# shgaurav1/DVG

Measured on AMD Instinct MI355X. Metric: predicted frames/sec at 64x64, batch 64, 10-in/10-out, higher is better.
Workload: dtype f32; 1 GPU; Moving-MNIST 64x64 rollout (generate_frames.py make_gifs sample loop), vgg_64 + lstm + GP trigger sample at i%15==0, batch 64 per GPU, 10-in/10-out; model_family=vgg, batch_per_gpu=64, n_past=10, n_future=10, parallelism=replicas x1 (no data-path collective), launch=hipGraph replay, rollouts_in_flight=3, tile_policy=energy, loop_invariant_skip_halves=hoisted, upsample_conv3x3=as transposed 4x4/s2 conv, conv3x3_deep_layers=Winograd F(4x4,3x3) / F(2x2,3x3)

## Files before the change

### dvg_amd/csrc/conv_igemm2.hip

```cpp
#include <cstdlib>
#include <type_traits>

#include "dvg_common.h"

namespace dvg {

constexpr int DVG_GEMM_WGS_PER_CU = DVG_BF16X3 ? 3 : 4;
constexpr int DVG_GEMM128_WGS = DVG_BF16X3 ? 3 : 2;
constexpr int DVG_GEMM128_GT = DVG_BF16X3 ? 2 : 4;
constexpr int DVG_GEMM_GT = 4;
constexpr int DVG_GEMM128_MIN_WGS = 4 * 768;
[[maybe_unused]] constexpr int DVG_GEMM_NT2 = 256;
constexpr int DVG_TILE16_MIN_WGS = 256;

enum { M2_CONV3 = 0, M2_CONV4S2 = 1, M2_CONVT4S2 = 2, M2_GEMM = 3 };

struct Igemm2Params {
    const float* x = nullptr;
    const float* skip = nullptr;
    const float* w = nullptr;
    const float* scale = nullptr;
    const float* shift = nullptr;
    float* y = nullptr;
    float* y_pool = nullptr;
    float* stats = nullptr;
    int N = 0, H = 0, W = 0, C1 = 0, C2 = 0, Cout = 0, upsample = 0, act = 0;
    float slope = 0.f;
    int tiles_y = 0, tiles_x = 0, tiles_n = 0, nblk_n = 0;
    int splitk = 1;
    int cps = 0;
    float* ws = nullptr;
    const float* addend = nullptr;
    unsigned long long* clk = nullptr;
    unsigned clk_cap = 0;
    int nb_group = 0;
    int stage_prio = 0;
    long w_image_stride = 0;
    int gemm_ni = 0;
    const int* add_map = nullptr;
    int add_B = 0;
    const float* first_frame = nullptr;
    const float* first_w = nullptr;
    const float* first_scale = nullptr;
    const float* first_shift = nullptr;
    float first_slope = 0.f;
    int y_from = 0;
    const float* proj_w = nullptr;
    float* proj_out = nullptr;
    int proj_T = 0;
};

__device__ __forceinline__ int addend_image(const int* __restrict__ add_map, int add_B, int n) {
    return add_map ? add_map[n / add_B] * add_B + n % add_B : n;
}

static unsigned long long* g_clk = nullptr;
static unsigned g_clk_cap = 0;

__device__ __attribute__((aligned(16))) float dvg_zero_slot[4] = {0.f, 0.f, 0.f, 0.f};

template <int MODE, int TI, int TH, int TW, int NT_ = 1, bool FIRST_ = false, bool PROJ_ = false>
struct Cfg2 {
    static constexpr int NT = NT_;
    static constexpr bool FIRST = FIRST_;
    static constexpr bool PROJ = PROJ_;
    static constexpr bool GEMM = MODE == M2_GEMM;
    static constexpr int S = (MODE == M2_CONV4S2) ? 2 : 1;
    static constexpr bool PAR4 = MODE == M2_CONV4S2;
    static constexpr int SPAN = GEMM ? 1 : (PAR4 ? 2 : 3);
    static constexpr int HH = (TH - 1) + SPAN, HW = (TW - 1) + SPAN;
    static constexpr bool LAYOUT = !GEMM;
    static constexpr int HWP = !LAYOUT ? HW : (TW == 16 ? HW : (TW == 8 ? 12 : 6));
    static constexpr int IMG = (LAYOUT && TI == 4) ? (PAR4 ? 30 : 40) : HH * HWP;
    static_assert(IMG >= HH * HWP && HWP >= HW, "halo layout");
    static constexpr int HP = TI * IMG;
    static constexpr unsigned P0PACK = !LAYOUT ? 0x6420u
        : (PAR4 ? (TW == 16 ? 0x3650u : (TI == 4 ? 0x7430u : 0x6530u))
                : (TW == 16 ? 0x2640u : (TI == 4 ? 0x6530u : 0x4620u)));
    static constexpr int PK = !LAYOUT ? 1 : (PAR4 ? (TW == 16 ? 4 : 1) : (TW == 16 ? 5 : (TI == 4 ? 1 : 3)));
    static constexpr bool STORE_PERM = LAYOUT && DVG_BF16X3 != 0;
    static constexpr int hp_of(int slot) {
        return STORE_PERM ? ((slot & ~7) | (((slot & 3) << 1) | ((slot >> 2) & 1))) : slot;
    }
    static constexpr int row_c(int reg) { return 4 * (int)((P0PACK >> (4 * (reg >> 2))) & 15u) + (reg & 3); }
    static constexpr int BM = TI * TH * TW, MT = BM / 64, BN = 64 * NT;
    static constexpr int NTAPS = GEMM ? 1 : ((MODE == M2_CONV3) ? 9 : 16);
    static constexpr int GT = (MODE == M2_CONV3) ? 9 : (MODE == M2_CONV4S2 ? 4 : (GEMM ? (NT == 2 ? 2 : (BM == 128 ? DVG_GEMM128_GT : DVG_GEMM_GT)) : 4));
    static constexpr int NG = (MODE == M2_CONV4S2) ? 16 / GT : 1;
    static constexpr int CHUNKS_PER_STAGE = GEMM ? GT : 1;
    static constexpr bool X3 = DVG_BF16X3 != 0;
    static constexpr int KC = 16, LD = X3 ? (GEMM ? 24 : 28) : 20, LDB = X3 ? 24 : 20, WROW = DVG_WROW;
    static constexpr int NP = X3 ? 3 : 2, PSTEP = X3 ? 8 : 4;
    static constexpr int BLK4 = GT * 64 * WROW / 4;
    static constexpr int B_TILE4 = NT * BLK4;
    static constexpr int NLB = (B_TILE4 + 255) / 256;
    static_assert(NT == 1 || (DVG_BF16X3 != 0 && MODE == M2_GEMM && BLK4 % 256 == 0), "NT = 2: bf16-triple GEMM mode only");
    static constexpr int NLA1 = (HP * 4 + 255) / 256;
    static constexpr int NLA = NLA1 * (GEMM ? GT : 1);
    static constexpr int SLAB = NLA1 * 64 * LD;
    static constexpr int A_FLOATS = NLA * 64 * LD, B_FLOATS = GT * BN * LDB;
    static constexpr int FP_W = HW + 2, FP_FLOATS = (HH + 2) * FP_W, FIRST_FLOATS = FIRST ? FP_FLOATS : 0;
    static_assert(!FIRST || (MODE == M2_CONV3 && TI == 1 && NT == 1), "FIRST: 3x3 mode, one image per tile");
    static constexpr int LDS_BYTES = (A_FLOATS + B_FLOATS + FIRST_FLOATS) * 4;
    static constexpr bool CAN_SPLIT = !FIRST && !GEMM && TW != 16 && !PROJ;
    static_assert(BM == 64 || BM == 128 || BM == 256, "BM");
    static_assert(!PROJ || (MODE == M2_CONVT4S2 && TI == 1 && NT == 1 && !FIRST && BM * 64 <= A_FLOATS + B_FLOATS),
                  "PROJ: transposed-conv mode, one image per tile, the staged tile fits the stage buffers");
};

template <int MODE, int TI, int TH, int TW, int NT = 1, bool FIRST = false, bool PROJ = false>
__global__ __launch_bounds__(256, (MODE == M2_GEMM && TW == 8) ? DVG_GEMM_WGS_PER_CU : ((MODE == M2_GEMM && NT == 1) ? DVG_GEMM128_WGS : 2)) void conv_igemm2_kernel(const Igemm2Params p) {
    using C = Cfg2<MODE, TI, TH, TW, NT, FIRST, PROJ>;
    constexpr int S = C::S, HH = C::HH, HW = C::HW, HP = C::HP, LD = C::LD, MT = C::MT, GT = C::GT, NG = C::NG,
                  BN = C::BN, NLA = C::NLA, NLA1 = C::NLA1, LDB = C::LDB, NP = C::NP, PSTEP = C::PSTEP, NLB = C::NLB;
    constexpr bool GEMM = C::GEMM, X3 = C::X3;
    extern __shared__ __attribute__((aligned(16))) float smem[];
    float* As = smem;
    float* Bs = smem + C::A_FLOATS;

    const int tid = threadIdx.x, lane = tid & 63, wave = tid >> 6;
    const int wm = wave >> 1, wn = wave & 1, l31 = lane & 31, hh = lane >> 5;

    unsigned lid = xcd_remap(blockIdx.x, gridDim.x);
    int par = 0;
    if (MODE == M2_CONVT4S2) { par = lid & 3; lid >>= 2; }
    const int split = lid % p.splitk;
    lid /= p.splitk;
    const int tiles_total = p.tiles_x * p.tiles_y * p.tiles_n;
    const unsigned lr = lid / p.nb_group;
    const int nb = (int)(lr / tiles_total) * p.nb_group + (int)(lid % p.nb_group);
    const unsigned tile_id = lr % tiles_total;
    unsigned t = tile_id;
    const int tx_i = t % p.tiles_x; t /= p.tiles_x;
    const int ty_i = t % p.tiles_y; t /= p.tiles_y;
    const int n0 = (int)t * (MODE == M2_GEMM ? p.gemm_ni : TI), y0 = ty_i * TH, x0 = tx_i * TW;
    const int yin0 = y0 * S - (GEMM ? 0 : 1), xin0 = x0 * S - (GEMM ? 0 : 1), nb0 = nb * BN;
    const float* const wbase = p.w + (GEMM ? (size_t)n0 * p.w_image_stride : 0);
    const int py = par >> 1, px = par & 1;
    const int Cin = p.C1 + p.C2;

    int a_base[MT];
#pragma unroll
    for (int mt = 0; mt < MT; ++mt) {
        const int lp = 4 * ((int)((C::P0PACK >> (4 * (l31 >> 3))) & 15u) ^ (((l31 >> 2) & 1) * C::PK)) + (l31 & 3);
        const int m = wm * (C::BM / 2) + mt * 32 + lp;
        const int ti = m / (TH * TW), r = m % (TH * TW);
        const int pos = ti * C::IMG + (r / TW) * C::HWP + r % TW;
        a_base[mt] = pos * LD + (X3 ? (hh ^ (GEMM ? (pos >> 3) & 1 : 0)) * 4 : hh * 8);
    }
    int b_base[NT];
#pragma unroll
    for (int nt = 0; nt < NT; ++nt) {
        const int col = (wn * NT + nt) * 32 + l31;
        b_base[nt] = ((col >> 6) * GT * 64 + (col & 63)) * LDB + (X3 ? (hh ^ ((l31 >> 3) & 1)) * 4 : hh * 8);
    }

    f32x16 acc[MT * NT];
#pragma unroll
    for (int mt = 0; mt < MT * NT; ++mt)
#pragma unroll
        for (int i = 0; i < 16; ++i) acc[mt][i] = 0.f;

    constexpr int NOFF = GEMM ? NLA1 : NLA;
    using aoff_t = typename std::conditional<GEMM || C::PAR4, int, long>::type;
    auto opaque = [](unsigned v) { asm("" : "+v"(v)); return v; };
    aoff_t offx[NOFF], offs[GEMM ? 1 : NLA];
    unsigned okmask = 0;
    static_assert(!C::PAR4 || NLA <= 4, "PAR4: four validity bits and two step bits per halo slot in one word");
    if (GEMM) offs[0] = 0;
#pragma unroll
    for (int i = 0; i < NLA; ++i) {
        const int idx = tid + (i % NLA1) * 256;
        const int hp = C::hp_of(idx >> 2), q = idx & 3;
        const int ti = hp / C::IMG, r = hp % C::IMG;
        const int hy = r / C::HWP, hx = r % C::HWP;
        const bool slot = hp < HP && hy < HH && hx < HW;
        if constexpr (C::PAR4) {
            const int n = n0 + ti, yy = yin0 + 2 * hy, xx = xin0 + 2 * hx;
            const bool in = slot && n < p.N;
#pragma unroll
            for (int par_ = 0; par_ < 4; ++par_) {
                const bool ok = in && (unsigned)(yy + (par_ >> 1)) < (unsigned)p.H && (unsigned)(xx + (par_ & 1)) < (unsigned)p.W;
                okmask |= ok ? (1u << (par_ * NLA + i)) : 0u;
            }
            const int cy0 = min(max(yy, 0), p.H - 1), cy1 = min(max(yy + 1, 0), p.H - 1);
            const int cx0 = min(max(xx, 0), p.W - 1), cx1 = min(max(xx + 1, 0), p.W - 1);
            okmask |= (in && cy1 != cy0) ? (1u << (16 + i)) : 0u;
            okmask |= (in && cx1 != cx0) ? (1u << (24 + i)) : 0u;
            offx[i] = in ? (int)((((long)n * p.H + cy0) * p.W + cx0) * p.C1 + q * 4) : 0;
            offs[i] = 0;
        } else {
        const int n = n0 + ti, yy = yin0 + hy, xx = xin0 + hx;
        const bool ok = slot && n < p.N && (unsigned)yy < (unsigned)p.H && (unsigned)xx < (unsigned)p.W;
        const int sh = p.upsample;
        okmask |= ok ? (1u << i) : 0u;
        if (!GEMM || i < NLA1)
            offx[GEMM ? i % NLA1 : i] = (aoff_t)(ok ? ((((long)(GEMM ? 0 : n) * (p.H >> sh) + (yy >> sh)) * (p.W >> sh) + (xx >> sh)) * p.C1 + q * 4) : 0);
        if (!GEMM) offs[i] = (ok && p.C2) ? ((((long)n * p.H + yy) * p.W + xx) * p.C2 + q * 4) : 0;
        }
    }
    auto tap_lds = [&](int grp, int tt) -> int {
        if (GEMM) return tt * C::SLAB;
        int th, tw;
        if (MODE == M2_CONV3) { th = tt / 3; tw = tt % 3; }
        else if (MODE == M2_CONV4S2) { th = tt >> 1; tw = tt & 1; }
        else { th = 1 + py - (tt >> 1); tw = 1 + px - (tt & 1); }
        return (th * C::HWP + tw) * LD;
    };
    long ld_a_off = GEMM ? (long)n0 * p.H * p.W * p.C1 : 0;
    const float* ld_w = wbase;
    float* const Fp = smem + C::A_FLOATS + C::B_FLOATS;
    f32x4 fw[FIRST ? 11 : 1];
    auto first_tile = [&](f32x4 (&ra)[NLA]) {
        if constexpr (FIRST) {
#pragma unroll
            for (int i = 0; i < NLA; ++i) {
                const int hp = min(C::hp_of((tid + i * 256) >> 2), HP - 1);
                const float* f = Fp + (hp / C::HWP) * C::FP_W + hp % C::HWP;
                f32x4 v = {0.f, 0.f, 0.f, 0.f};
#pragma unroll
                for (int t = 0; t < 9; ++t) {
                    const float px = f[(t / 3) * C::FP_W + t % 3];
#pragma unroll
                    for (int e = 0; e < 4; ++e) v[e] = fmaf(fw[t][e], px, v[e]);
                }
                const float okf = (float)((okmask >> i) & 1u);
#pragma unroll
                for (int e = 0; e < 4; ++e) {
                    const float a = v[e] * fw[9][e] + fw[10][e];
                    v[e] = fmaxf(a, a * p.first_slope) * okf;
                }
                ra[i] = v;
            }
        }
    };
    auto gload_a = [&](int c0, f32x4 (&ra)[NLA], const int par_ = 0) {
        if constexpr (FIRST) {
            const float* w = p.first_w + c0 + (tid & 3) * 4;
#pragma unroll
            for (int t = 0; t < 9; ++t) fw[t] = *reinterpret_cast<const f32x4*>(w + t * 64);
            fw[9] = *reinterpret_cast<const f32x4*>(p.first_scale + c0 + (tid & 3) * 4);
            fw[10] = *reinterpret_cast<const f32x4*>(p.first_shift + c0 + (tid & 3) * 4);
            return;
        }
        const bool from_x = GEMM || c0 < p.C1;
        const float* src = (from_x ? p.x + c0 : p.skip + (c0 - p.C1)) + (GEMM ? ld_a_off : 0);
#pragma unroll
        for (int i = 0; i < NLA; ++i) {
            if (GEMM) {
                ra[i] = *reinterpret_cast<const f32x4*>(src + offx[i % NLA1] + (i / NLA1) * 16);
            } else if (C::PAR4) {
                int off = offx[i];
                if (par_ >> 1) off += (int)opaque((okmask >> (16 + i)) & 1u) * (p.W * p.C1);
                if (par_ & 1) off += (int)opaque((okmask >> (24 + i)) & 1u) * p.C1;
                ra[i] = *reinterpret_cast<const f32x4*>(src + off);
            } else {
                const float* a = src + (from_x ? offx[GEMM ? 0 : i] : offs[GEMM ? 0 : i]);
                ra[i] = *reinterpret_cast<const f32x4*>(((okmask >> i) & 1u) ? a : dvg_zero_slot);
            }
        }
    };
    auto gload_b = [&](int chunk, int grp, f32x4 (&rb)[NLB]) {
        const float* tile;
        if (GEMM) tile = ld_w + ((size_t)nb * NT * (Cin / C::KC) + chunk) * (64 * C::WROW);
        else tile = wbase + (((size_t)chunk * (p.Cout >> 6) + nb) * C::NTAPS + (MODE == M2_CONVT4S2 ? par * 4 : grp * GT)) * (64 * C::WROW);
#pragma unroll
        for (int j = 0; j < NLB; ++j) {
            int i = tid + j * 256;
            if (C::B_TILE4 % 256) i = min(i, C::B_TILE4 - 1);
            const size_t blk = (NT > 1 && j * 256 >= C::BLK4) ? (size_t)(Cin / C::KC) * (64 * C::WROW / 4) - C::BLK4 : 0;
            rb[j] = reinterpret_cast<const f32x4*>(tile)[i + blk];
        }
    };
    auto lds_store_a = [&](f32x4 (&ra)[NLA], const int par_ = 0) {
        if constexpr (FIRST) first_tile(ra);
#pragma unroll
        for (int i = 0; i < NLA; ++i) {
            const int idx = tid + (i % NLA1) * 256;
            const int hp = C::hp_of(idx >> 2), q = idx & 3;
            if constexpr (C::PAR4) {
                const unsigned keep = 0u - opaque((okmask >> (par_ * NLA + i)) & 1u);
#pragma unroll
                for (int e = 0; e < 4; ++e) {
                    const float f = ra[i][e];
                    ra[i][e] = __builtin_bit_cast(float, __builtin_bit_cast(unsigned, f) & keep);
                }
            }
            if constexpr (X3) {
                u32x2_t h, m, l;
                unsigned t0, t1, t2;
                bf16x3_split_pair(ra[i][0], ra[i][1], t0, t1, t2);
                h[0] = t0; m[0] = t1; l[0] = t2;
                bf16x3_split_pair(ra[i][2], ra[i][3], t0, t1, t2);
                h[1] = t0; m[1] = t1; l[1] = t2;
                float* d = &As[(i / NLA1) * C::SLAB + hp * LD + ((q >> 1) ^ (GEMM ? (hp >> 3) & 1 : 0)) * 4 + (q & 1) * 2];
                *reinterpret_cast<u32x2_t*>(d) = h;
                *reinterpret_cast<u32x2_t*>(d + 8) = m;
                *reinterpret_cast<u32x2_t*>(d + 16) = l;
            } else {
                *reinterpret_cast<f32x4*>(&As[(i / NLA1) * C::SLAB + hp * LD + q * 4]) = ra[i];
            }
        }
    };
    auto lds_store_b = [&](const f32x4 (&rb)[NLB]) {
#pragma unroll
        for (int j = 0; j < NLB; ++j) {
            int i = tid + j * 256;
            if (C::B_TILE4 % 256) i = min(i, C::B_TILE4 - 1);
            if constexpr (X3) reinterpret_cast<f32x4*>(Bs)[i] = rb[j];
            else *reinterpret_cast<f32x4*>(&Bs[(i >> 2) * LDB + (i & 3) * 4]) = rb[j];
        }
    };

    constexpr int CPS = C::CHUNKS_PER_STAGE;
    const int chunk_begin = split * p.cps;
    const int chunk_end = min(Cin / C::KC, chunk_begin + p.cps);
    f32x4 ra[NLA], rb[NLB];
    unsigned long long clk0 = 0, wclk0 = 0;
    if (p.clk) {
        clk0 = clock64();
        wclk0 = wall_clock64();
    }
    if constexpr (FIRST) {
        const float* fr = p.first_frame + (size_t)n0 * p.H * p.W;
        for (int i = tid; i < C::FP_FLOATS; i += 256) {
            const int yy = yin0 - 1 + i / C::FP_W, xx = xin0 - 1 + i % C::FP_W;
            Fp[i] = ((unsigned)yy < (unsigned)p.H && (unsigned)xx < (unsigned)p.W) ? fr[(size_t)yy * p.W + xx] : 0.f;
        }
        __syncthreads();
    }
    gload_a(chunk_begin * C::KC, ra);
    gload_b(chunk_begin, 0, rb);
    lds_store_a(ra);
    lds_store_b(rb);
    __syncthreads();
    unsigned long long clk1 = 0;
    if (p.clk) clk1 = clock64();

    auto stage = [&](const int chunk, auto grp_c, auto has_next_c, const int nchunk_override = -1) __attribute__((always_inline)) {
        constexpr int grp = decltype(grp_c)::value;
        constexpr bool has_next = decltype(has_next_c)::value;
        constexpr int ngrp = (grp + 1) % NG;
        constexpr bool next_a = has_next && (ngrp == 0 || C::PAR4);
        const int nchunk = nchunk_override >= 0 ? nchunk_override : chunk + (ngrp == 0 ? CPS : 0);
        if constexpr (next_a) gload_a(nchunk * C::KC, ra, C::PAR4 ? ngrp : 0);
        if constexpr (has_next) gload_b(nchunk, ngrp, rb);

        f32x4 fa[2][MT][NP], fb[2][NT][NP];
        {
            const int ao = tap_lds(grp, 0);
#pragma unroll
            for (int j = 0; j < NP; ++j) {
#pragma unroll
                for (int mt = 0; mt < MT; ++mt)
                    fa[0][mt][j] = *reinterpret_cast<const f32x4*>(&As[a_base[mt] + ao + j * PSTEP]);
#pragma unroll
                for (int nt = 0; nt < NT; ++nt)
                    fb[0][nt][j] = *reinterpret_cast<const f32x4*>(&Bs[b_base[nt] + j * PSTEP]);
            }
        }
#pragma unroll
        for (int tt = 0; tt < GT; ++tt) {
            const int cur = tt & 1, nxt = cur ^ 1;
            constexpr bool LEAN = X3 && (NT == 2 || (GEMM && MT == 2));
            auto read_plane = [&](int j) {
                const int ao = tap_lds(grp, tt + 1);
#pragma unroll
                for (int mt = 0; mt < MT; ++mt)
                    fa[nxt][mt][j] = *reinterpret_cast<const f32x4*>(&As[a_base[mt] + ao + j * PSTEP]);
#pragma unroll
                for (int nt = 0; nt < NT; ++nt)
                    fb[nxt][nt][j] = *reinterpret_cast<const f32x4*>(&Bs[b_base[nt] + (tt + 1) * 64 * LDB + j * PSTEP]);
            };
            if (LEAN && tt + 1 < GT) read_plane(0);
            if (!LEAN && tt + 1 < GT) {
                const int ao = tap_lds(grp, tt + 1);
#pragma unroll
                for (int j = 0; j < NP; ++j) {
#pragma unroll
                    for (int mt = 0; mt < MT; ++mt)
                        fa[nxt][mt][j] = *reinterpret_cast<const f32x4*>(&As[a_base[mt] + ao + j * PSTEP]);
#pragma unroll
                    for (int nt = 0; nt < NT; ++nt)
                        fb[nxt][nt][j] = *reinterpret_cast<const f32x4*>(&Bs[b_base[nt] + (tt + 1) * 64 * LDB + j * PSTEP]);
                }
            }
            if (has_next && tt == GT - 1) {
                __syncthreads();
                if constexpr (next_a) lds_store_a(ra, C::PAR4 ? ngrp : 0);
                lds_store_b(rb);
            }
            if constexpr (X3) {
                auto mm = [&](int pa, int pb) {
#pragma unroll
                    for (int mt = 0; mt < MT; ++mt)
#pragma unroll
                        for (int nt = 0; nt < NT; ++nt)
                            acc[mt * NT + nt] = __builtin_amdgcn_mfma_f32_32x32x16_bf16(
                                __builtin_bit_cast(bf16x8_t, fa[cur][mt][pa]), __builtin_bit_cast(bf16x8_t, fb[cur][nt][pb]),
                                acc[mt * NT + nt], 0, 0, 0);
                };
                if constexpr (LEAN) {
                    mm(2, 0);
                    mm(0, 2);
                    if (tt + 1 < GT) read_plane(2);
                    mm(1, 1);
                    mm(1, 0);
                    mm(0, 1);
                    if (tt + 1 < GT) read_plane(1);
                    mm(0, 0);
                } else {
                    mm(2, 0);
                    mm(1, 1);
                    mm(0, 2);
                    mm(1, 0);
                    mm(0, 1);
                    mm(0, 0);
                }
            } else {
#pragma unroll
                for (int j = 0; j < 2; ++j)
#pragma unroll
                    for (int e = 0; e < 4; ++e)
#pragma unroll
                        for (int mt = 0; mt < MT; ++mt)
                            acc[mt] = __builtin_amdgcn_mfma_f32_32x32x2f32(fa[cur][mt][j][e], fb[cur][0][j][e], acc[mt], 0, 0, 0);
            }
            constexpr int NREAD = NP * (MT + NT), NMFMA = (X3 ? 6 : 8) * MT * NT, MPR = NMFMA >= 2 * NREAD ? 2 : 1;
            constexpr int NVMEM = (next_a ? (FIRST ? 11 : NLA) : 0) + (has_next ? NLB : 0);
            constexpr int VT0 = GT >= 9 ? 2 : 0;
            constexpr int SLOTS = (GT - 1 - VT0) > 0 ? (GT - 1 - VT0) : 1;
            constexpr int VNEED = (NVMEM + SLOTS - 1) / SLOTS;
            constexpr int VPT = VNEED > 2 ? VNEED : 2;
            constexpr int VTAPS = (NVMEM + VPT - 1) / VPT;
            if (tt == 0) __builtin_amdgcn_sched_group_barrier(0x100, NREAD, 0);
            if (LEAN && tt + 1 < GT) {
                constexpr int G = MT * NT, R = MT + NT;
#pragma unroll
                for (int r = 0; r < R; ++r) {
                    __builtin_amdgcn_sched_group_barrier(0x100, 1, 0);
                    __builtin_amdgcn_sched_group_barrier(0x008, 1, 0);
                }
                __builtin_amdgcn_sched_group_barrier(0x008, 2 * G - R, 0);
#pragma unroll
                for (int r = 0; r < R; ++r) {
                    __builtin_amdgcn_sched_group_barrier(0x100, 1, 0);
                    __builtin_amdgcn_sched_group_barrier(0x008, 1, 0);
                }
                __builtin_amdgcn_sched_group_barrier(0x008, 3 * G - R, 0);
#pragma unroll
                for (int r = 0; r < R; ++r) {
                    __builtin_amdgcn_sched_group_barrier(0x100, 1, 0);
                    __builtin_amdgcn_sched_group_barrier(0x008, 1, 0);
                }
            } else if (tt + 1 < GT) {
#pragma unroll
                for (int r = 0; r < NREAD; ++r) {
                    __builtin_amdgcn_sched_group_barrier(0x100, 1, 0);
                    __builtin_amdgcn_sched_group_barrier(0x008, MPR, 0);
                }
                if (NMFMA > MPR * NREAD) __builtin_amdgcn_sched_group_barrier(0x008, NMFMA - MPR * NREAD, 0);
            } else if (has_next) {
                constexpr int NW = (next_a ? NLA * (X3 ? 3 : 1) : 0) + NLB;
#pragma unroll
                for (int r = 0; r < NW; ++r) {
                    if (r < NMFMA) __builtin_amdgcn_sched_group_barrier(0x008, 1, 0);
                    __builtin_amdgcn_sched_group_barrier(0x200, 1, 0);
                }
                if (NMFMA > NW) __builtin_amdgcn_sched_group_barrier(0x008, NMFMA - NW, 0);
            } else {
                __builtin_amdgcn_sched_group_barrier(0x008, NMFMA, 0);
            }
            if (tt >= VT0 && tt < VT0 + VTAPS && tt + 1 < GT) __builtin_amdgcn_sched_group_barrier(0x020, VPT, 0);
        }

        if constexpr (has_next) __syncthreads();
    };
    using std::integral_constant;
    const bool prio_on = p.stage_prio != 0;
    auto set_prio = [&](int st) {
        if (!prio_on) return;
        switch (st & 3) {
            case 0: __builtin_amdgcn_s_setprio(3); break;
            case 1: __builtin_amdgcn_s_setprio(2); break;
            case 2: __builtin_amdgcn_s_setprio(1); break;
            default: __builtin_amdgcn_s_setprio(0); break;
        }
    };
    int chunk = chunk_begin, st = 0;
    if constexpr (GEMM) {
        const int spi = (chunk_end - chunk_begin) / CPS;
        const long a_img = (long)p.H * p.W * p.C1;
        const unsigned lane_off = (unsigned)(4 * hh * p.Cout + l31);
        float* const ybase = p.y + (size_t)n0 * p.H * p.W * p.Cout + nb0 + __builtin_amdgcn_readfirstlane(wn) * 32 * NT;
        const int wm_u = __builtin_amdgcn_readfirstlane(wm);
        for (int img = 0; img < p.gemm_ni; ++img) {
            for (int sg = 0; sg < spi; ++sg) {
                const bool wrap = sg == spi - 1, last = wrap && img == p.gemm_ni - 1;
                ld_a_off = (long)(n0 + img + (wrap ? 1 : 0)) * a_img;
                ld_w = wbase + (size_t)(img + (wrap ? 1 : 0)) * p.w_image_stride;
                const int nchunk = wrap ? chunk_begin : chunk_begin + (sg + 1) * CPS;
                set_prio(st++);
                if (last) stage(chunk_begin + sg * CPS, integral_constant<int, 0>{}, integral_constant<bool, false>{});
                else stage(chunk_begin + sg * CPS, integral_constant<int, 0>{}, integral_constant<bool, true>{}, nchunk);
            }
            float* const yb = ybase + (size_t)img * p.H * p.W * p.Cout;
#pragma unroll
            for (int mt = 0; mt < MT; ++mt) {
                const int mbase = wm_u * (C::BM / 2) + mt * 32;
#pragma unroll
                for (int nt = 0; nt < NT; ++nt)
#pragma unroll
                    for (int reg = 0; reg < 16; ++reg) {
                        const int mu = mbase + (reg & 3) + 8 * (reg >> 2);
                        float* const dst = (yb + (size_t)((y0 + mu / TW) * p.W + x0 + mu % TW) * p.Cout + nt * 32) + lane_off;
                        *dst = acc[mt * NT + nt][reg];
                        acc[mt * NT + nt][reg] = 0.f;
                    }
            }
        }
    } else {
    auto chunk_stages = [&](const int ch, auto last_c) __attribute__((always_inline)) {
        constexpr bool last = decltype(last_c)::value;
        set_prio(st++);
        stage(ch, integral_constant<int, 0>{}, integral_constant<bool, !(last && NG == 1)>{});
        if constexpr (NG >= 2) {
            set_prio(st++);
            stage(ch, integral_constant<int, 1>{}, integral_constant<bool, !(last && NG == 2)>{});
        }
        if constexpr (NG >= 4) {
            set_prio(st++);
            stage(ch, integral_constant<int, 2>{}, integral_constant<bool, true>{});
            set_prio(st++);
            stage(ch, integral_constant<int, 3>{}, integral_constant<bool, !last>{});
        }
        static_assert(NG == 1 || NG == 2 || NG == 4, "stages per chunk");
    };
    for (; chunk + CPS < chunk_end; chunk += CPS) chunk_stages(chunk, integral_constant<bool, false>{});
    chunk_stages(chunk, integral_constant<bool, true>{});
    }
    __builtin_amdgcn_s_setprio(0);
    unsigned long long clk_loop = 0;
    if (p.clk) clk_loop = clock64();
    auto clk_exit = [&]() {
        if (p.clk && threadIdx.x == 0 && blockIdx.x < p.clk_cap) {
            unsigned long long* d = p.clk + (size_t)blockIdx.x * 8;
            d[0] = clk0; d[1] = clk1; d[2] = clk_loop; d[3] = clock64(); d[4] = wclk0; d[5] = wall_clock64();
            unsigned xcc;
            asm volatile("s_getreg_b32 %0, hwreg(HW_REG_XCC_ID)" : "=s"(xcc));
            unsigned hwid;
            asm volatile("s_getreg_b32 %0, hwreg(HW_REG_HW_ID)" : "=s"(hwid));
            d[6] = xcc; d[7] = hwid;
        }
    };

    if constexpr (GEMM) {
        clk_exit();
        return;
    }
    int Ho, Wo;
    if (MODE == M2_CONV3 || MODE == M2_GEMM) { Ho = p.H; Wo = p.W; }
    else if (MODE == M2_CONV4S2) { Ho = p.H >> 1; Wo = p.W >> 1; }
    else { Ho = p.H * 2; Wo = p.W * 2; }
    const int c = nb0 + wn * 32 + l31;
    if (C::CAN_SPLIT && p.splitk > 1) {
        const size_t slab = (size_t)p.N * Ho * Wo * p.Cout;
        float* const wsp = p.ws + (size_t)split * slab;
#pragma unroll
        for (int mt = 0; mt < MT; ++mt)
#pragma unroll
            for (int reg = 0; reg < 16; ++reg) {
                const int m = wm * (C::BM / 2) + mt * 32 + (C::row_c(reg) ^ (hh * 4 * C::PK));
                const int tii = m / (TH * TW), r = m % (TH * TW);
                const int ty = r / TW, tx = r % TW;
                const int n = n0 + tii;
                int oy, ox;
                if (MODE == M2_CONVT4S2) { oy = 2 * (y0 + ty) + py; ox = 2 * (x0 + tx) + px; }
                else { oy = y0 + ty; ox = x0 + tx; }
                if (n < p.N) wsp[(((size_t)n * Ho + oy) * Wo + ox) * p.Cout + c] = acc[mt][reg];
            }
        clk_exit();
        return;
    }
    const float sc = p.scale ? p.scale[c] : 1.f, sf = p.shift ? p.shift[c] : 0.f;
    float s1 = 0.f, s2 = 0.f;
    float* const yb = p.y + (size_t)n0 * Ho * Wo * p.Cout + c;
    const bool want_y = !FIRST || n0 >= p.y_from;
    float* const pb = p.y_pool ? p.y_pool + (size_t)n0 * (Ho >> 1) * (Wo >> 1) * p.Cout + c : nullptr;
    const float* const ab = p.addend ? p.addend + (size_t)n0 * Ho * Wo * p.Cout + c : nullptr;
    long add_shift[TI];
#pragma unroll
    for (int t_ = 0; t_ < TI; ++t_) {
        const int n_ = min(n0 + t_, p.N - 1);
        add_shift[t_] = (ab != nullptr && p.add_map != nullptr)
                            ? (long)(addend_image(p.add_map, p.add_B, n_) - n_) * Ho * Wo * p.Cout : 0;
    }
    auto shift_of = [&](int tii) -> long {
        if (TI == 1) return add_shift[0];
        long v = add_shift[0];
#pragma unroll
        for (int t_ = 1; t_ < TI; ++t_) v = tii == t_ ? add_shift[t_] : v;
        return v;
    };
    const int hrow = hh * 4 * C::PK;
    [[maybe_unused]] float* const Ps = smem;
    [[maybe_unused]] constexpr int PNT = 3;
    [[maybe_unused]] const int i16 = lane & 15, kq = lane >> 4;
    [[maybe_unused]] f32x4 pw[PROJ ? PNT : 1][PROJ ? 4 : 1];
    constexpr bool PW_EARLY = TW == 16;
    auto load_pw = [&]() {
        if constexpr (PROJ) {
#pragma unroll
            for (int nt = 0; nt < PNT; ++nt)
#pragma unroll
                for (int j = 0; j < 4; ++j)
                    pw[nt][j] = *reinterpret_cast<const f32x4*>(p.proj_w + min(nt * 16 + i16, p.proj_T - 1) * 64 + 16 * j + 4 * kq);
        }
    };
    if constexpr (PROJ) {
        if (PW_EARLY) load_pw();
        __syncthreads();
    }
    auto epilogue = [&](auto act_c) {
        constexpr int ACT = decltype(act_c)::value;
#pragma unroll
        for (int mt = 0; mt < MT; ++mt) {
            float v[16];
            const int mbase = wm * (C::BM / 2) + mt * 32;
            const int ti0 = mbase / (TH * TW);
            if (ab != nullptr) {
                float av[16];
#pragma unroll
                for (int reg = 0; reg < 16; ++reg) {
                    const int m = mbase + (C::row_c(reg) ^ hrow);
                    const int tii = (TH * TW >= 32) ? ti0 : m / (TH * TW);
                    const int r = m % (TH * TW);
                    const int ty = r / TW, tx = r % TW;
                    int oy, ox;
                    if (MODE == M2_CONVT4S2) { oy = 2 * (y0 + ty) + py; ox = 2 * (x0 + tx) + px; }
                    else { oy = y0 + ty; ox = x0 + tx; }
                    av[reg] = (TI == 1 || n0 + tii < p.N) ? ab[(long)((tii * Ho + oy) * Wo + ox) * p.Cout + shift_of(tii)] : 0.f;
                }
#pragma unroll
                for (int reg = 0; reg < 16; ++reg) v[reg] = (acc[mt][reg] + av[reg]) * sc + sf;
            } else {
#pragma unroll
                for (int reg = 0; reg < 16; ++reg) v[reg] = acc[mt][reg] * sc + sf;
            }
#pragma unroll
            for (int reg = 0; reg < 16; ++reg) {
                const int row = C::row_c(reg) ^ hrow;
                const int m = mbase + row;
                const int tii = (TH * TW >= 32) ? ti0 : m / (TH * TW);
                const int r = m % (TH * TW);
                const int ty = r / TW, tx = r % TW;
                if (TI == 1 || n0 + tii < p.N) {
                    s1 += v[reg];
// ... 141 lines not shown
            }
            if (addend != nullptr) {
                size_t aoff = off;
                if (add_map != nullptr) {
                    const long img4 = (long)H * W * C4;
                    const int n_ = (int)(off / img4);
                    aoff = off - (size_t)(n_ - addend_image(add_map, add_B, n_)) * img4;
                }
                const f32x4 t = reinterpret_cast<const f32x4*>(addend)[aoff];
#pragma unroll
                for (int k = 0; k < 4; ++k) v[k] += t[k];
            }
#pragma unroll
            for (int k = 0; k < 4; ++k) {
                const float u = v[k] * sc[k] + sf[k];
                s1[k] += u;
                s2[k] = fmaf(u, u, s2[k]);
                v[k] = apply_act(u, act, slope);
            }
            reinterpret_cast<f32x4*>(y)[off] = v;
            if (POOL) {
                if (q == 0) mx = v;
                else
#pragma unroll
                    for (int k = 0; k < 4; ++k) mx[k] = fmaxf(mx[k], v[k]);
            }
        }
        if (POOL) reinterpret_cast<f32x4*>(y_pool)[w_ * C4 + c4] = mx;
    }
    if (stats != nullptr) {
#pragma unroll
        for (int k = 0; k < 4; ++k) {
            red[(tp * TC + tc) * 4 + k] = s1[k];
            red[1024 + (tp * TC + tc) * 4 + k] = s2[k];
        }
        __syncthreads();
        if (tp == 0) {
            float* dst = stats + (size_t)blockIdx.x * 2 * C;
#pragma unroll
            for (int k = 0; k < 4; ++k) {
                float a = 0.f, b = 0.f;
                for (int r = 0; r < TP; ++r) {
                    a += red[(r * TC + tc) * 4 + k];
                    b += red[1024 + (r * TC + tc) * 4 + k];
                }
                dst[c4 * 4 + k] = a;
                dst[C + c4 * 4 + k] = b;
            }
        }
    }
}

static int finish_units_per_block(long units) {
    long upb = (units + 1023) / 1024;
    if (upb < 8) upb = 8;
    return (int)upb;
}

static int g_tile_policy = 0;
extern "C" void dvg_set_tile_policy(int energy) { g_tile_policy = energy ? 1 : 0; }
extern "C" int dvg_tile_policy(void) { return g_tile_policy; }

static int choose_splitk(long wgs, int nchunks) {
    if (wgs >= 384 || nchunks < 8) return 1;
    long s = 512 / wgs;
    if (s > 8) s = 8;
    if (s > nchunks / 4) s = nchunks / 4;
    if (s < 2) return 1;
    const int cps = (int)((nchunks + s - 1) / s);
    return (nchunks + cps - 1) / cps;
}

static int gemm_images_per_wg(int tw, int nt, int NB, int Hg, int Wg, int Cout) {
#if DVG_BF16X3
    if (tw == 8 && nt == 1) {
        const long w1 = (long)(Hg / 8) * (Wg / 8) * NB * (Cout / 64), slots = 256L * DVG_GEMM_WGS_PER_CU;
        if (w1 % slots == 0 && w1 / slots >= 2 && w1 / slots <= 6 && NB % (w1 / slots) == 0) return (int)(w1 / slots);
    }
#endif
    return 1;
}

static int choose_nb_group(long tiles, int nblk_n, double wb, double ib) {
    const double per_xcd = (double)tiles * nblk_n / 8.0;
    int best = nblk_n;
    double cost = 1e300;
    for (int a = 1; a <= nblk_n; ++a) {
        if (nblk_n % a) continue;
        const double share_tiles = per_xcd / a;
        if (share_tiles > (double)tiles) continue;
        const double c = a * wb + (share_tiles < 1.0 ? 1.0 : share_tiles) * ib;
        if (c < cost) { cost = c; best = a; }
    }
    return best;
}

constexpr bool can_split2(int mode, int tw, bool fused) { return mode != M2_GEMM && tw != 16 && !fused; }

struct Plan2 {
    int ti, th, tw, nt, ni;
    int Hg, Wg, Ho, Wo;
    int ty, tx, tn;
    long tiles, wgs;
    bool can_split, pool;
    int splitk, cps;
    long units;
    int upb, fgrid;
    int stats_rows;
};

static int plan2(Plan2* pl, int mode, int N, int H, int W, int Cin, int Cout, bool with_ws, bool pool, bool fused = false,
                 int n_tile = 0) {
    Plan2 q{};
    const int par = mode == M2_CONVT4S2 ? 4 : 1, sh = mode == M2_CONV4S2 ? 2 : 1;
    q.Hg = H / sh; q.Wg = W / sh;
    q.Ho = mode == M2_CONVT4S2 ? 2 * H : q.Hg; q.Wo = mode == M2_CONVT4S2 ? 2 * W : q.Wg;
    q.ti = 1; q.th = 8; q.tw = 8; q.nt = 1; q.ni = 1;
    if (q.Hg == 4 && q.Wg == 4) {
        q.ti = q.th = q.tw = 4;
    } else if (q.Hg % 8 || q.Wg % 8) {
        return -1;
    } else if (q.Wg % 16 == 0) {
        const long w16 = (long)(n_tile ? n_tile : N) * (q.Hg / 8) * (q.Wg / 16) * par;
        if (w16 * (Cout / 64) >= (g_tile_policy ? DVG_TILE16_MIN_WGS : 512)) q.tw = 16;
        if (mode == M2_GEMM && q.tw == 16 && (!DVG_BF16X3 || w16 * (Cout / 64) < DVG_GEMM128_MIN_WGS)) q.tw = 8;
        if (mode == M2_GEMM && DVG_BF16X3 && g_tile_policy && Cout % 128 == 0 && w16 * (Cout / 128) >= DVG_GEMM_NT2) { q.tw = 16; q.nt = 2; }
    }
    if (mode == M2_GEMM && q.ti != 1) return -1;
    if (mode == M2_GEMM) q.ni = gemm_images_per_wg(q.tw, q.nt, N, q.Hg, q.Wg, Cout);
    q.ty = q.Hg / q.th; q.tx = q.Wg / q.tw; q.tn = mode == M2_GEMM ? N / q.ni : (N + q.ti - 1) / q.ti;
    q.tiles = (long)q.ty * q.tx * q.tn * par;
    q.wgs = q.tiles * (Cout / (64 * q.nt));
    q.can_split = can_split2(mode, q.tw, fused); q.pool = pool;
    q.splitk = (with_ws && q.can_split) ? choose_splitk(q.wgs, Cin / 16) : 1;
    q.cps = (Cin / 16 + q.splitk - 1) / q.splitk;
    q.units = pool ? (long)N * (q.Ho / 2) * (q.Wo / 2) : (long)N * q.Ho * q.Wo;
    q.upb = finish_units_per_block(q.units);
    q.fgrid = (int)((q.units + q.upb - 1) / q.upb);
    q.stats_rows = q.splitk > 1 ? q.fgrid : (int)q.tiles;
    *pl = q;
    return 0;
}

template <int TI_, int TH_, int TW_, int NT_ = 1>
struct Tile2 { static constexpr int TI = TI_, TH = TH_, TW = TW_, NT = NT_; };

template <int MODE, class T, bool FIRST = false, bool PROJ = false>
static int launch2(Igemm2Params p, const Plan2& pl, float* ws, long ws_floats, hipStream_t stream) {
    constexpr int TI = T::TI, TH = T::TH, TW = T::TW, NT = T::NT;
    using C = Cfg2<MODE, TI, TH, TW, NT, FIRST, PROJ>;
    static_assert(C::CAN_SPLIT == can_split2(MODE, TW, FIRST || PROJ), "the host's split rule is the kernels'");
    if (pl.ti != TI || pl.th != TH || pl.tw != TW || pl.nt != NT || pl.can_split != C::CAN_SPLIT || pl.pool != (p.y_pool != nullptr))
        return fail(DVG_ERR_SHAPE, "conv_igemm2: the plan is not this launch's");
    if (pl.Hg % TH || pl.Wg % TW || p.Cout % C::BN || pl.cps % C::CHUNKS_PER_STAGE)
        return fail(DVG_ERR_SHAPE, "conv_igemm2: tile does not divide shape");
    p.tiles_y = pl.ty; p.tiles_x = pl.tx; p.tiles_n = pl.tn;
    if (MODE == M2_GEMM) p.gemm_ni = pl.ni;
    p.nblk_n = p.Cout / C::BN;
    p.clk = g_clk; p.clk_cap = g_clk_cap;
    p.nb_group = choose_nb_group((long)p.tiles_y * p.tiles_x * p.tiles_n, p.nblk_n,
                                 (double)C::NTAPS * (p.C1 + p.C2) * C::BN * 4, (double)C::BM * (p.C1 + p.C2) * 4);
    const int S = pl.splitk;
    if (S > 1 && (long)S * p.N * pl.Ho * pl.Wo * p.Cout > ws_floats) return fail(DVG_ERR_SHAPE, "conv_igemm2: split-K workspace too small");
    p.cps = pl.cps; p.splitk = S; p.ws = ws;
    const unsigned grid = (unsigned)(pl.wgs * S);
    p.stage_prio = (MODE == M2_CONV3 || grid <= 3 * 256) ? 1 : 0;
    static bool attr_set = false;
    if (!attr_set) {
        hipError_t e = hipFuncSetAttribute(reinterpret_cast<const void*>(&conv_igemm2_kernel<MODE, TI, TH, TW, NT, FIRST, PROJ>),
                                           hipFuncAttributeMaxDynamicSharedMemorySize, C::LDS_BYTES);
        if (e != hipSuccess) return fail(DVG_ERR_HIP, "hipFuncSetAttribute: %s", hipGetErrorString(e));
        attr_set = true;
    }
    hipLaunchKernelGGL((conv_igemm2_kernel<MODE, TI, TH, TW, NT, FIRST, PROJ>), dim3(grid), dim3(256), C::LDS_BYTES, stream, p);
    if (int e = check_launch("conv_igemm2")) return e;
    if (S == 1) return DVG_OK;
    auto finish = pl.pool ? splitk_finish_kernel<true> : splitk_finish_kernel<false>;
    hipLaunchKernelGGL(finish, dim3(pl.fgrid), dim3(256), 0, stream, ws, S, p.scale, p.shift, p.y, p.y_pool, p.stats, p.N, pl.Ho,
                       pl.Wo, p.Cout, p.act, p.slope, pl.upb, p.addend, p.add_map, p.add_B);
    return check_launch("splitk_finish");
}

enum { T2_444 = 1, T2_NT2 = 2 };
template <int MODE, int EXTRA = 0, bool PROJ = false>
static int launch_tile(const Igemm2Params& p, const Plan2& pl, const char* who, float* ws, long ws_floats, void* stream) {
    auto go = [&](auto t) { return launch2<MODE, decltype(t), false, PROJ>(p, pl, ws, ws_floats, (hipStream_t)stream); };
    if constexpr ((EXTRA & T2_NT2) != 0 && DVG_BF16X3 != 0)
        if (pl.ti == 1 && pl.tw == 16 && pl.nt == 2) return go(Tile2<1, 8, 16, 2>{});
    if constexpr ((EXTRA & T2_444) != 0)
        if (pl.ti == 4 && pl.nt == 1) return go(Tile2<4, 4, 4>{});
    if (pl.ti == 1 && pl.tw == 16 && pl.nt == 1) return go(Tile2<1, 8, 16>{});
    if (pl.ti == 1 && pl.tw == 8 && pl.nt == 1) return go(Tile2<1, 8, 8>{});
    return fail(DVG_ERR_SHAPE, "%s: no kernel", who);
}


#if DVG_BF16X3
struct CfgWX {
    static constexpr int TH = 8, TP = 8, TW = 2 * TP, HH = TH + 2, HW = TW + 2, HP = HH * HW;
    static constexpr int LD = 28, LDB = 24, WROW = DVG_WROW;
    static constexpr int PLANE = HH * TP * LD + 8;
    static constexpr int A_FLOATS = 4 * PLANE, B_FLOATS = 4 * 64 * LDB;
    static constexpr int NLB = 4 * 64 * WROW / 4 / 256;
    static constexpr int ND = (HP * 4 + 255) / 256;
    static constexpr int D_FLOATS = ND * 64 * 16;
    static constexpr int NX = 4 * HH * TP * 4 / 256;
    static constexpr int FP_W = HW + 2, FP_FLOATS = (HH + 2) * FP_W;
    static constexpr int lds_bytes(bool first) { return (A_FLOATS + B_FLOATS + D_FLOATS + (first ? FP_FLOATS : 0)) * 4; }
    static_assert(4 * HH * TP * 4 % 256 == 0 && 4 * 64 * WROW / 4 % 256 == 0, "whole passes");
};

template <bool FIRST>
__global__ __launch_bounds__(256, 2) void conv3_wx_kernel(const Igemm2Params p) {
    using C = CfgWX;
    constexpr int LD = C::LD, LDB = C::LDB, NLB = C::NLB, ND = C::ND, NX = C::NX;
    extern __shared__ __attribute__((aligned(16))) float smem[];
    float* const As = smem;
    float* const Bs = As + C::A_FLOATS;
    float* const Ds = Bs + C::B_FLOATS;
    float* const Fp = Ds + C::D_FLOATS;

    const int tid = threadIdx.x, lane = tid & 63, wave = tid >> 6;
    const int wm = wave >> 1, wn = wave & 1, l31 = lane & 31, hh = lane >> 5;

    const unsigned lid = xcd_remap(blockIdx.x, gridDim.x);
    const int tiles_total = p.tiles_x * p.tiles_y * p.tiles_n;
    const unsigned lr = lid / p.nb_group;
    const int nb = (int)(lr / tiles_total) * p.nb_group + (int)(lid % p.nb_group);
    unsigned t = lr % tiles_total;
    const int tx_i = t % p.tiles_x; t /= p.tiles_x;
    const int ty_i = t % p.tiles_y; t /= p.tiles_y;
    const int n0 = (int)t, y0 = ty_i * C::TH, x0 = tx_i * C::TW, yin0 = y0 - 1, xin0 = x0 - 1, nb0 = nb * 64;

    const int a_base = (wm * 32 + l31) * LD + hh * 4;
    const int b_base = (wn * 32 + l31) * LDB + (hh ^ ((l31 >> 3) & 1)) * 4;

    f32x16 acc[4];
#pragma unroll
    for (int f = 0; f < 4; ++f)
#pragma unroll
        for (int i = 0; i < 16; ++i) acc[f][i] = 0.f;

    long offx[FIRST ? 1 : ND];
    unsigned okmask = 0;
#pragma unroll
    for (int i = 0; i < ND; ++i) {
        const int hp = (tid + i * 256) >> 2;
        const int yy = yin0 + hp / C::HW, xx = xin0 + hp % C::HW;
        const bool ok = hp < C::HP && (unsigned)yy < (unsigned)p.H && (unsigned)xx < (unsigned)p.W;
        okmask |= ok ? (1u << i) : 0u;
        if constexpr (!FIRST) offx[i] = ok ? (((long)n0 * p.H + yy) * p.W + xx) * p.C1 + (tid & 3) * 4 : 0;
    }
    const int xf = (tid >> 2) & 3, xq = tid & 3;
    const int x_ia = xf == 0 ? 0 : (xf == 2 ? 2 : 1), x_ib = xf == 2 ? 1 : (xf == 3 ? 3 : 2);
    const float x_sg = xf == 1 ? 1.f : -1.f;
    const int x_pix = (tid >> 7) * C::HW + 2 * ((tid >> 4) & 7);
    const int x_da = (x_pix + x_ia) * 16 + xq * 4, x_db = (x_pix + x_ib) * 16 + xq * 4;
    const int x_st = xf * C::PLANE + (tid >> 4) * LD + (xq >> 1) * 4 + (xq & 1) * 2;

    f32x4 fw[FIRST ? 11 : 1];
    f32x4 ra[ND], rb[NLB];
    auto gload_d = [&](int c0) {
        if constexpr (FIRST) {
            const float* w = p.first_w + c0 + (tid & 3) * 4;
#pragma unroll
            for (int tp = 0; tp < 9; ++tp) fw[tp] = *reinterpret_cast<const f32x4*>(w + tp * 64);
            fw[9] = *reinterpret_cast<const f32x4*>(p.first_scale + c0 + (tid & 3) * 4);
            fw[10] = *reinterpret_cast<const f32x4*>(p.first_shift + c0 + (tid & 3) * 4);
        } else {
            const float* src = p.x + c0;
#pragma unroll
            for (int i = 0; i < ND; ++i)
                ra[i] = *reinterpret_cast<const f32x4*>(((okmask >> i) & 1u) ? src + offx[i] : dvg_zero_slot);
        }
    };
    auto store_d = [&]() {
        if constexpr (FIRST) {
#pragma unroll
            for (int i = 0; i < ND; ++i) {
                const int hp = min((tid + i * 256) >> 2, C::HP - 1);
                const float* f = Fp + (hp / C::HW) * C::FP_W + hp % C::HW;
                f32x4 v = {0.f, 0.f, 0.f, 0.f};
#pragma unroll
                for (int tp = 0; tp < 9; ++tp) {
                    const float px = f[(tp / 3) * C::FP_W + tp % 3];
#pragma unroll
                    for (int e = 0; e < 4; ++e) v[e] = fmaf(fw[tp][e], px, v[e]);
                }
                const float okf = (float)((okmask >> i) & 1u);
#pragma unroll
                for (int e = 0; e < 4; ++e) {
                    const float a = v[e] * fw[9][e] + fw[10][e];
                    v[e] = fmaxf(a, a * p.first_slope) * okf;
                }
                ra[i] = v;
            }
        }
#pragma unroll
        for (int i = 0; i < ND; ++i) reinterpret_cast<f32x4*>(Ds)[tid + i * 256] = ra[i];
    };
    auto gload_b = [&](int chunk, int r) {
        const float* tile = p.w + (((size_t)chunk * (p.Cout >> 6) + nb) * 12 + r * 4) * (64 * C::WROW);
#pragma unroll
        for (int j = 0; j < NLB; ++j) rb[j] = reinterpret_cast<const f32x4*>(tile)[tid + j * 256];
    };
    auto store_b = [&]() {
// ... 536 lines not shown
```

Measured before the change: 52320 frames/s.

## Stream GEMM weight fragments from global into registers for NT=2 bf16x3 tiles

```diff
diff --git a/dvg_amd/csrc/conv_igemm2.hip b/dvg_amd/csrc/conv_igemm2.hip
--- a/dvg_amd/csrc/conv_igemm2.hip
+++ b/dvg_amd/csrc/conv_igemm2.hip
@@ -98,7 +98,8 @@
     static constexpr int NLA1 = (HP * 4 + 255) / 256;
     static constexpr int NLA = NLA1 * (GEMM ? GT : 1);
     static constexpr int SLAB = NLA1 * 64 * LD;
-    static constexpr int A_FLOATS = NLA * 64 * LD, B_FLOATS = GT * BN * LDB;
+    static constexpr bool WREG = X3 && GEMM && NT == 2;
+    static constexpr int A_FLOATS = NLA * 64 * LD, B_FLOATS = WREG ? 0 : GT * BN * LDB;
     static constexpr int FP_W = HW + 2, FP_FLOATS = (HH + 2) * FP_W, FIRST_FLOATS = FIRST ? FP_FLOATS : 0;
     static_assert(!FIRST || (MODE == M2_CONV3 && TI == 1 && NT == 1), "FIRST: 3x3 mode, one image per tile");
     static constexpr int LDS_BYTES = (A_FLOATS + B_FLOATS + FIRST_FLOATS) * 4;
@@ -272,6 +273,18 @@
             rb[j] = reinterpret_cast<const f32x4*>(tile)[i + blk];
         }
     };
+    [[maybe_unused]] f32x4 bq[C::WREG ? 2 : 1][NT][NP];
+    constexpr int BQ_SLAB = 64 * C::WROW * (int)sizeof(float);
+    [[maybe_unused]] const char* bq_ptr = reinterpret_cast<const char*>(wbase)
+        + (((size_t)nb * NT + wn) * (Cin / C::KC) + split * p.cps) * BQ_SLAB + (l31 * LDB + (hh ^ ((l31 >> 3) & 1)) * 4) * (int)sizeof(float);
+    [[maybe_unused]] auto gload_bq = [&](const int buf) __attribute__((always_inline)) {
+#pragma unroll
+        for (int nt = 0; nt < NT; ++nt)
+#pragma unroll
+            for (int j = 0; j < NP; ++j)
+                bq[buf][nt][j] = *reinterpret_cast<const f32x4*>(bq_ptr + (nt * 32 * LDB + j * PSTEP) * (int)sizeof(float));
+        bq_ptr += BQ_SLAB;
+    };
     auto lds_store_a = [&](f32x4 (&ra)[NLA], const int par_ = 0) {
         if constexpr (FIRST) first_tile(ra);
 #pragma unroll
@@ -330,9 +343,10 @@
         __syncthreads();
     }
     gload_a(chunk_begin * C::KC, ra);
-    gload_b(chunk_begin, 0, rb);
+    if constexpr (C::WREG) gload_bq(0);
+    else gload_b(chunk_begin, 0, rb);
     lds_store_a(ra);
-    lds_store_b(rb);
+    if constexpr (!C::WREG) lds_store_b(rb);
     __syncthreads();
     unsigned long long clk1 = 0;
     if (p.clk) clk1 = clock64();
@@ -343,8 +357,8 @@
         constexpr int ngrp = (grp + 1) % NG;
         constexpr bool next_a = has_next && (ngrp == 0 || C::PAR4);
         const int nchunk = nchunk_override >= 0 ? nchunk_override : chunk + (ngrp == 0 ? CPS : 0);
-        if constexpr (next_a) gload_a(nchunk * C::KC, ra, C::PAR4 ? ngrp : 0);
-        if constexpr (has_next) gload_b(nchunk, ngrp, rb);
+        if constexpr (next_a && !C::WREG) gload_a(nchunk * C::KC, ra, C::PAR4 ? ngrp : 0);
+        if constexpr (has_next && !C::WREG) gload_b(nchunk, ngrp, rb);
 
         f32x4 fa[2][MT][NP], fb[2][NT][NP];
         {
@@ -354,6 +368,7 @@
 #pragma unroll
                 for (int mt = 0; mt < MT; ++mt)
                     fa[0][mt][j] = *reinterpret_cast<const f32x4*>(&As[a_base[mt] + ao + j * PSTEP]);
+                if constexpr (!C::WREG)
 #pragma unroll
                 for (int nt = 0; nt < NT; ++nt)
                     fb[0][nt][j] = *reinterpret_cast<const f32x4*>(&Bs[b_base[nt] + j * PSTEP]);
@@ -362,12 +377,18 @@
 #pragma unroll
         for (int tt = 0; tt < GT; ++tt) {
             const int cur = tt & 1, nxt = cur ^ 1;
+            static_assert(!C::WREG || GT % 2 == 0, "WREG: slab parity = buffer parity across stages");
+            if constexpr (C::WREG) {
+                if (tt + 1 < GT || has_next) gload_bq(nxt);
+                if constexpr (next_a) if (tt == 0) gload_a(nchunk * C::KC, ra, 0);
+            }
             constexpr bool LEAN = X3 && (NT == 2 || (GEMM && MT == 2));
             auto read_plane = [&](int j) {
                 const int ao = tap_lds(grp, tt + 1);
 #pragma unroll
                 for (int mt = 0; mt < MT; ++mt)
                     fa[nxt][mt][j] = *reinterpret_cast<const f32x4*>(&As[a_base[mt] + ao + j * PSTEP]);
+                if constexpr (!C::WREG)
 #pragma unroll
                 for (int nt = 0; nt < NT; ++nt)
                     fb[nxt][nt][j] = *reinterpret_cast<const f32x4*>(&Bs[b_base[nt] + (tt + 1) * 64 * LDB + j * PSTEP]);
@@ -388,16 +409,20 @@
             if (has_next && tt == GT - 1) {
                 __syncthreads();
                 if constexpr (next_a) lds_store_a(ra, C::PAR4 ? ngrp : 0);
-                lds_store_b(rb);
+                if constexpr (!C::WREG) lds_store_b(rb);
             }
             if constexpr (X3) {
+                auto bfrag = [&](int nt, int pb) -> f32x4 {
+                    if constexpr (C::WREG) return bq[cur][nt][pb];
+                    else return fb[cur][nt][pb];
+                };
                 auto mm = [&](int pa, int pb) {
 #pragma unroll
                     for (int mt = 0; mt < MT; ++mt)
 #pragma unroll
                         for (int nt = 0; nt < NT; ++nt)
                             acc[mt * NT + nt] = __builtin_amdgcn_mfma_f32_32x32x16_bf16(
-                                __builtin_bit_cast(bf16x8_t, fa[cur][mt][pa]), __builtin_bit_cast(bf16x8_t, fb[cur][nt][pb]),
+                                __builtin_bit_cast(bf16x8_t, fa[cur][mt][pa]), __builtin_bit_cast(bf16x8_t, bfrag(nt, pb)),
                                 acc[mt * NT + nt], 0, 0, 0);
                 };
                 if constexpr (LEAN) {
@@ -426,16 +451,17 @@
                         for (int mt = 0; mt < MT; ++mt)
                             acc[mt] = __builtin_amdgcn_mfma_f32_32x32x2f32(fa[cur][mt][j][e], fb[cur][0][j][e], acc[mt], 0, 0, 0);
             }
-            constexpr int NREAD = NP * (MT + NT), NMFMA = (X3 ? 6 : 8) * MT * NT, MPR = NMFMA >= 2 * NREAD ? 2 : 1;
-            constexpr int NVMEM = (next_a ? (FIRST ? 11 : NLA) : 0) + (has_next ? NLB : 0);
+            constexpr int NREAD = NP * (MT + (C::WREG ? 0 : NT)), NMFMA = (X3 ? 6 : 8) * MT * NT, MPR = NMFMA >= 2 * NREAD ? 2 : 1;
+            constexpr int NVMEM = (next_a ? (FIRST ? 11 : NLA) : 0) + (has_next && !C::WREG ? NLB : 0);
             constexpr int VT0 = GT >= 9 ? 2 : 0;
             constexpr int SLOTS = (GT - 1 - VT0) > 0 ? (GT - 1 - VT0) : 1;
             constexpr int VNEED = (NVMEM + SLOTS - 1) / SLOTS;
             constexpr int VPT = VNEED > 2 ? VNEED : 2;
             constexpr int VTAPS = (NVMEM + VPT - 1) / VPT;
             if (tt == 0) __builtin_amdgcn_sched_group_barrier(0x100, NREAD, 0);
+            if (C::WREG && (tt + 1 < GT || has_next)) __builtin_amdgcn_sched_group_barrier(0x020, NT * NP, 0);
             if (LEAN && tt + 1 < GT) {
-                constexpr int G = MT * NT, R = MT + NT;
+                constexpr int G = MT * NT, R = MT + (C::WREG ? 0 : NT);
 #pragma unroll
                 for (int r = 0; r < R; ++r) {
                     __builtin_amdgcn_sched_group_barrier(0x100, 1, 0);
@@ -453,6 +479,7 @@
                     __builtin_amdgcn_sched_group_barrier(0x100, 1, 0);
                     __builtin_amdgcn_sched_group_barrier(0x008, 1, 0);
                 }
+                if (G > R) __builtin_amdgcn_sched_group_barrier(0x008, G - R, 0);
             } else if (tt + 1 < GT) {
 #pragma unroll
                 for (int r = 0; r < NREAD; ++r) {
@@ -461,7 +488,7 @@
                 }
                 if (NMFMA > MPR * NREAD) __builtin_amdgcn_sched_group_barrier(0x008, NMFMA - MPR * NREAD, 0);
             } else if (has_next) {
-                constexpr int NW = (next_a ? NLA * (X3 ? 3 : 1) : 0) + NLB;
+                constexpr int NW = (next_a ? NLA * (X3 ? 3 : 1) : 0) + (C::WREG ? 0 : NLB);
 #pragma unroll
                 for (int r = 0; r < NW; ++r) {
                     if (r < NMFMA) __builtin_amdgcn_sched_group_barrier(0x008, 1, 0);
@@ -494,15 +521,25 @@
         const unsigned lane_off = (unsigned)(4 * hh * p.Cout + l31);
         float* const ybase = p.y + (size_t)n0 * p.H * p.W * p.Cout + nb0 + __builtin_amdgcn_readfirstlane(wn) * 32 * NT;
         const int wm_u = __builtin_amdgcn_readfirstlane(wm);
-        for (int img = 0; img < p.gemm_ni; ++img) {
-            for (int sg = 0; sg < spi; ++sg) {
-                const bool wrap = sg == spi - 1, last = wrap && img == p.gemm_ni - 1;
-                ld_a_off = (long)(n0 + img + (wrap ? 1 : 0)) * a_img;
-                ld_w = wbase + (size_t)(img + (wrap ? 1 : 0)) * p.w_image_stride;
-                const int nchunk = wrap ? chunk_begin : chunk_begin + (sg + 1) * CPS;
+        const int ni = C::WREG ? 1 : p.gemm_ni;
+        for (int img = 0; img < ni; ++img) {
+            if constexpr (C::WREG) {
+                for (int sg = 0; sg + 1 < spi; ++sg) {
+                    set_prio(st++);
+                    stage(chunk_begin + sg * CPS, integral_constant<int, 0>{}, integral_constant<bool, true>{}, chunk_begin + (sg + 1) * CPS);
+                }
                 set_prio(st++);
-                if (last) stage(chunk_begin + sg * CPS, integral_constant<int, 0>{}, integral_constant<bool, false>{});
-                else stage(chunk_begin + sg * CPS, integral_constant<int, 0>{}, integral_constant<bool, true>{}, nchunk);
+                stage(chunk_begin + (spi - 1) * CPS, integral_constant<int, 0>{}, integral_constant<bool, false>{});
+            } else {
+                for (int sg = 0; sg < spi; ++sg) {
+                    const bool wrap = sg == spi - 1, last = wrap && img == p.gemm_ni - 1;
+                    ld_a_off = (long)(n0 + img + (wrap ? 1 : 0)) * a_img;
+                    ld_w = wbase + (size_t)(img + (wrap ? 1 : 0)) * p.w_image_stride;
+                    const int nchunk = wrap ? chunk_begin : chunk_begin + (sg + 1) * CPS;
+                    set_prio(st++);
+                    if (last) stage(chunk_begin + sg * CPS, integral_constant<int, 0>{}, integral_constant<bool, false>{});
+                    else stage(chunk_begin + sg * CPS, integral_constant<int, 0>{}, integral_constant<bool, true>{}, nchunk);
+                }
             }
             float* const yb = ybase + (size_t)img * p.H * p.W * p.Cout;
 #pragma unroll
@@ -950,6 +987,7 @@
     static_assert(C::CAN_SPLIT == can_split2(MODE, TW, FIRST || PROJ), "the host's split rule is the kernels'");
     if (pl.ti != TI || pl.th != TH || pl.tw != TW || pl.nt != NT || pl.can_split != C::CAN_SPLIT || pl.pool != (p.y_pool != nullptr))
         return fail(DVG_ERR_SHAPE, "conv_igemm2: the plan is not this launch's");
+    if (C::WREG && pl.ni != 1) return fail(DVG_ERR_SHAPE, "conv_igemm2: the 128 x 128 tile runs one image per workgroup");
     if (pl.Hg % TH || pl.Wg % TW || p.Cout % C::BN || pl.cps % C::CHUNKS_PER_STAGE)
         return fail(DVG_ERR_SHAPE, "conv_igemm2: tile does not divide shape");
     p.tiles_y = pl.ty; p.tiles_x = pl.tx; p.tiles_n = pl.tn;
```

Result: faster. 53470 frames/s, median of 6 (+2.2%).
